# bioinformatics-centre/BayesTyper

Hardware: AMD Instinct MI355X
Metric: variant-cluster Gibbs iterations/sec + k-mer matches/sec at 1/2/4/8 MI355X (higher is better)
Workload: dtype f64 log-probabilities over u8 k-mer counts (Gibbs); u64/u8 integer (k-mer matching)

## Files before the change

bayestyper_amd/csrc/bt_gibbs.hip:

```cpp
#ifndef BT_SWEEP_OUTLINE
#define BT_SWEEP_INLINE
#endif
#include "bt_genotypes.hpp"
#include "bt_gibbs_kernel.hpp"
#include "bt_gibbs_timeline.hpp"
#include "bt_internal.hpp"

#include <algorithm>
#include <atomic>
#include <chrono>
#include <cmath>
#include <cstring>
#include <map>
#include <memory>
#include <numeric>

using namespace bt;

namespace bt {
hipError_t launch_gibbs_simple_kernel(unsigned grid, uint32_t lds, hipStream_t st, const TileDesc *tiles, uint8_t *pool, const GParams *P, int op, uint32_t a0, uint32_t a1,
                                      unsigned long long *hist, TraceCfg tr, const uint32_t *tile_list, TimelineDev *tl);
hipError_t prepare_gibbs_simple_kernel(int max_lds);
hipError_t launch_gibbs_hot_kernel(unsigned grid, unsigned block, uint32_t lds, hipStream_t st, const TileDesc *tiles, uint8_t *pool, const GParams *P, int op, uint32_t a0, uint32_t a1,
                                   unsigned long long *hist, TraceCfg tr, const uint32_t *tile_list, TimelineDev *tl);
// ... 818 lines not shown
            BT_HIP(launch_gibbs_hot_kernel(c.pack_wgs, LANES * c.pack_waves, c.pack_lds, st, g->d_tiles, g->d_pool, g->d_params, op, a0, a1, hist, tr, (const uint32_t *)c.d_pack, tl));
        else if (tl)
            hipLaunchKernelGGL(gibbs_kernel_tl, dim3((unsigned)c.tiles.size()), dim3(LANES * c.split), c.lds, st, g->d_tiles, g->d_pool, g->d_params, op, a0, a1, hist, tr,
                               (const uint32_t *)c.d_tiles, tl);
        else
            hipLaunchKernelGGL(gibbs_kernel, dim3((unsigned)c.tiles.size()), dim3(LANES * c.split), c.lds, st, g->d_tiles, g->d_pool, g->d_params, op, a0, a1, hist, tr,
                               (const uint32_t *)c.d_tiles);
        BT_CHECK_LAUNCH();
        if (tl) tl += class_waves(c);
        if (wide && c.num_fill) {
            hipLaunchKernelGGL(nan_fill_kernel, dim3(c.num_fill), dim3(256), 0, st, g->d_pool, (const FillChunk *)c.d_fill);
            BT_CHECK_LAUNCH();
        }
        if (c.stream) BT_HIP(hipEventRecord(c.done, st));
    }
    for (auto &c : g->classes)
        if (c.stream) BT_HIP(hipStreamWaitEvent(g->ctx->stream, c.done, 0));
    g->prefill_armed = wide;
    return BT_OK;
}

inline uint64_t align_up(uint64_t x, uint64_t a) { return (x + a - 1) / a * a; }
inline uint32_t tile_lds_bytes(const TileDesc &d) { return d.lds_all ? d.hot_bytes * d.nvm : d.hot_bytes; }
constexpr uint32_t kMinTileWidth = 4;
constexpr uint32_t kLightLds = 24576;
const uint32_t kClassLds[] = {16384, 32768, 0xFFFFFFFFu};

const uint32_t kElemSize[A_COUNT] = {
     1,  1,  1,  1,  4,  4,  2,  4,  2,  4,  4,  4,  2,
     1,  4,  4,  4,  2,  4,  4,  4,  4,  4,  4,
     4,  1,
     4,  8,  8,  4,  4,  4,  4,  1,  2,  8,  4,  1,
     4,  4,  4,  4,  4,  4,  8,  4,  8,  2,  8,
     8,  4,  8,  1,  4,  4,  8,  1,  1,  8,  4,  8,  4,  1,  4,  8,  4,
     4,  1,  8,  4,  4,  4,  1,  1,  1,  1,  4,  2,  4,  8,  8,  4,  2,  1,  4,  4,  4,  1,  1,  1,  1,  4,  4};

}

extern "C" {

struct bt_gibbs_source {
    bt_ctx *ctx = nullptr;
    uint32_t S = 0, G = 0, C = 0;
    std::vector<ClusterDims> cd;
    std::vector<GroupDims> gd;
    BuildBatch dev{};
// ... 326 lines not shown
            for (uint32_t c = 0; c < x.nv; ++c) cd_sel.push_back(src->cd[c0 + c]);
            gd_sel[i] = x;
        }
        C = (uint32_t)cd_sel.size();
        cd = cd_sel.data();
        gd = gd_sel.data();
    }
    if (G == 0 || C == 0) return fail("bt_gibbs_create: empty batch");
    BT_HIP(hipSetDevice(ctx->device));
    bt_gibbs *g = new bt_gibbs();
    g->ctx = ctx;
    g->G = G;
    g->C = C;
    g->S = S;
    GParams &P = g->P;
    P.S = S;
    P.seed = params->seed;
    P.num_chains = params->num_chains;
    P.burn_in = params->burn_in;
    P.num_iterations = params->num_iterations;
    P.max_hvk = params->max_haplotype_variant_kmers;
    P.noise_seeding = params->noise_seeding;
    P.rate = (double)params->kmer_subsampling_rate;
    for (uint32_t s = 0; s < S; ++s) P.gender[s] = params->gender[s] ? 1 : 0;

#define BT_TRY(x)                \
    do {                         \
        int _rc = (x);           \
        if (_rc != BT_OK) {      \
            bt_gibbs_destroy(g); \
            return _rc;          \
        }                        \
    } while (0)
#define BT_TRYHIP(x)                                                     \
    do {                                                                 \
        hipError_t _e = (x);                                             \
        if (_e != hipSuccess) {                                          \
            bt_gibbs_destroy(g);                                         \
            return fail(std::string(#x) + ": " + hipGetErrorString(_e)); \
        }                                                                \
    } while (0)

    g->h_A.assign(C, 0);
    g->h_var_off.assign((size_t)C + 1, 0);
    for (uint32_t c = 0; c < C; ++c) g->h_var_off[c + 1] = g->h_var_off[c] + cd[c].V;
    uint64_t flat_sel = 0;
// ... 2061 lines not shown
            break;
        case 2:
            for (uint64_t i = 0; i < n; ++i) h_out[i] = rng_gamma(st, nd, a[i], b[i]);
            break;
        case 3:
            for (uint64_t i = 0; i < n; ++i) h_out[i] = (double)rng_uniform_int(st, (uint32_t)a[i] + 1u);
            break;
        case 4:
            for (uint64_t i = 0; i < n; ++i) h_out[i] = rng_bernoulli(st, (double)(float)a[0]) ? 1.0 : 0.0;
            break;
        case 5: {
            std::vector<uint32_t> v((size_t)a[0]);
            for (size_t i = 0; i < v.size(); ++i) v[i] = (uint32_t)i;
            rng_shuffle_u32(st, sptr1(v.data()), (uint32_t)v.size());
            for (size_t i = 0; i < v.size(); ++i) h_out[i] = v[i];
            break;
        }
        default:
            return fail("bt_diag_rng: unknown kind");
    }
    return BT_OK;
}

}
```

bayestyper_amd/csrc/bt_gibbs_kernel.hpp:

```cpp
#pragma once
#include "bt_gibbs_tile.hpp"
#include "bt_noise_chain.hpp"
#include "bt_noise_help.hpp"
#include "bt_gibbs_simple.hpp"

namespace bt {

enum GibbsOp { OP_RUN = 0, OP_INIT_CHAIN = 1, OP_SWEEP = 2, OP_NOISE = 3, OP_RESET = 4, OP_SETUP = 5, OP_NOISE_CHAIN = 6 };

struct TraceCfg {
    uint32_t max_sweeps;
    uint32_t *counter;
    uint32_t *buf;
};

__device__ BT_NOINLINE void group_init_chain(Env env, uint32_t chain, uint32_t nvert, uint32_t nsrc, uint32_t gindex) {
    const Tile t = make_tile(env);
    const GParams BT_CAS &P = env_params(env);
    const uint32_t gseed = P.noise_seeding ? P.seed + (gindex + 1u) * (chain + 1u) : P.seed + (gindex + 1u);
    for (uint32_t v = 0; v < nvert; ++v) {
        const Vx c = make_vx(t, v);
        Env ev = env;
        const bool swap = env.resident == 0xFFFFFFFFu && t.d->hot_bytes != 0;
        if (swap) {
            hot_swap(env, v, true);
            ev.resident = v;
        }
        PROF_DECL;
        if (!make_vx(make_tile(ev), v).sc()[SC_CONSTRUCTED]) genotyper_construct(ev, v, gseed + c.cid());
        genotyper_reset(ev, v);
        if (swap) hot_swap(env, v, false);
    }
    if (nvert == 1 && nsrc == 1) return;
    uint32_t *bst = (uint32_t *)(t.base + t.d->off[A_BRNG]) + (size_t)t.plane * MT_PAD;
    mt_seed(bst, P.seed + (gindex + 1u) * (chain + 1u));
    Mt brng = mt_open(bst);
    rng_shuffle_u32(brng, t.arr<uint32_t>(A_SOURCES), nsrc);
    for (uint32_t v = 0; v < nvert; ++v) {
        const Vx c = make_vx(t, v);
        rng_shuffle_u32(brng, c.edges(), vx_ne(c));
    }
}

__device__ BT_NOINLINE void prepare_nested(Env env, uint32_t v_parent, uint32_t v_child) {
    if (env.resident != RESIDENT_ALL && env.resident != RESIDENT_NEVER) env.resident = 0xFFFFFFFFu;
    const Tile t = make_tile(env);
    const GParams BT_CAS &P = env_params(env);
    const Vx c = make_vx(t, v_parent), cc = make_vx(t, v_child);
    const uint32_t nd_n = vx_nd(c), cc_cid = cc.cid();
    const TileDesc BT_CAS &d = c.d();
    TPtr<uint32_t> ndcl = c.a<uint32_t>(A_NDCL, d.NDm > 1 ? d.NDm : 1), ndvo = c.a<uint32_t>(A_NDVOFF, d.NDm + 1);
    TPtr<uint16_t> ndv = c.a<uint16_t>(A_NDVAR, d.NDVm > 1 ? d.NDVm : 1);
    TPtr<uint32_t> pver = c.nver(), cver = cc.nver();
// ... 189 lines not shown
    const NoiseChainCtl *nc = is_nc ? (const NoiseChainCtl *)hist : nullptr;
    const bool no_lds = is_nc && (t.d->lds_all ? t.d->hot_bytes * t.d->nvm : t.d->hot_bytes) > nc->lds_cap;
    if (no_lds) env.resident = t.resident = RESIDENT_NEVER;
    const bool whole = !no_lds && (t.d->nvm == 1 || t.d->lds_all) && t.d->hot_bytes != 0 && (op == OP_RUN || op == OP_SWEEP || op == OP_INIT_CHAIN || is_nc);
    if (whole) {
        env.resident = RESIDENT_ALL;
        for (uint32_t v = 0; v < nvert; ++v) hot_swap(env, v, true);
        t.resident = RESIDENT_ALL;
        t.hot = lds_block() + t.lds0;
    }
    const bool simple = SIMPLE_ONLY;
    if (op == OP_RUN || op == OP_SWEEP || is_nc) {
        const bool is_run = op == OP_RUN;
        const uint32_t nchains = is_run ? P.num_chains : 1u;
        uint32_t n_burn = is_run ? P.burn_in : (arg1 != 0 ? 0u : arg0), n_collect = is_run ? P.num_iterations : (arg1 != 0 ? arg0 : 0u);
        if (is_nc) {
            n_burn = nc->first_collect < nc->n_iterations ? nc->first_collect : nc->n_iterations;
            n_collect = nc->n_iterations - n_burn;
            if (!nc_begin(nc)) n_burn = n_collect = 0;
        }
        for (uint32_t chain = 0; chain < nchains; ++chain) {
            if (is_run) {
                PROF_DECL;
                group_init_chain(env, chain, nvert, nsrc, gindex);
                PROF(15);
            }
            if constexpr (SIMPLE_ONLY) {
                simple_sweeps(env, t, P, n_burn, n_collect, tr.counter, tr.buf, tr.max_sweeps, tile, nc);
                if (is_run || n_collect) drain_collected(env);
            } else {
                const uint32_t i0 = is_nc ? nc->it_begin : 0u;
                for (uint32_t i = i0; i < n_burn + n_collect; ++i) {
                    if (is_nc && i > i0) {
                        nc_phase(nc, 0x10000000u | i);
                        if (!nc_wait_table(nc, i)) break;
                        if (nc->help_units) {
                            noise_help(env, nc);
                            if (!noise_help_wait(nc, tile, i)) break;
                        }
                    }
                    if (is_nc) nc_phase(nc, 0x40000000u | i);
                    const TraceRow r = trace_row_for(t, P, tr, tile);
                    if constexpr (kSingle) {
                        if (r.on)
                            for (uint32_t q = 0; q < P.S; ++q) r.row[q] = 0xFFFFFFFFu;
                        const Vx root = make_vx(t, 0);
                        TPtr<uint8_t> gploidy = t.arr<uint8_t>(A_PLOIDY);
                        for (uint32_t q = 0; q < P.S; ++q) {
                            root.nest_ploidy()[q] = gploidy[q];
                            root.nest_n()[q] = 0;
                        }
                        visit_vertex(env, t, P, 0u, i >= n_burn, r.row, r.on);
                    } else
                        group_sweep(env, t, P, i >= n_burn, nvert, nsrc, r.row, r.on);
                    if (is_nc) {
                        nc_phase(nc, 0x50000000u | i);
                        noise_tally_group(env, nvert, nc);
                        nc_phase(nc, 0x60000000u | i);
                        if (!nc_iteration_end(nc, i)) break;
                    }
                }
                if (is_run && t.d->logged) drain_collected(env);
            }
        }
        if (!simple && (is_run || n_collect))
            for (uint32_t v = 0; v < nvert; ++v) flush_vertex(env, v);
    } else if (op == OP_INIT_CHAIN) {
        group_init_chain(env, arg0, nvert, nsrc, gindex);
        if (!SIMPLE_ONLY && arg1 != 0 && wide_table(*t.d))
            for (uint32_t v = 0; v < nvert; ++v) make_vx(t, v).sc()[SC_UC_DIRTY] = 0;
    } else if (SIMPLE_ONLY) {
    } else if (op == OP_NOISE) {
        for (uint32_t v = 0; v < nvert; ++v) {
            const Vx c = make_vx(t, v);
            const uint32_t nsu = c.sc()[SC_NSUB_U];
            TPtr<uint32_t> usub = c.usub();
            for (uint32_t s = 0; s < P.S; ++s) {
                const uint16_t h1 = c.dip()[2 * s], h2 = c.dip()[2 * s + 1];
                for (uint32_t i = t.part; i < nsu; i += t.copies) {
                    const uint32_t k = usub[i];
                    if (unique_mult(c, k, h1, h2, P.gender[s]) == 0) {
                        const uint32_t cnt = c.has_counts(k) ? c.count(k, s) : 0;
                        atomicAdd(&hist[s * 256u + cnt], 1ULL);
                    }
                }
            }
            if (t.part == 0) cache_clear(c, P, false, arg0 != 0);
        }
    } else if (op == OP_RESET) {
        for (uint32_t v = 0; v < nvert; ++v) make_vx(t, v).sc()[SC_CONSTRUCTED] = 0;
    } else if (op == OP_SETUP) {
// ... 36 lines not shown
```

bayestyper_amd/csrc/bt_gibbs_tile.hpp:

```cpp
#pragma once
#include "bt_rng_device.hpp"

namespace bt {

constexpr unsigned LANES = 64;
constexpr uint16_t NOHAP = 0xFFFF;
constexpr double BT_LN2 = 0.693147180559945309417232121458176568;
constexpr double BT_DBL_EPS = 2.220446049250313080847263336181640625e-16;
#ifndef BT_LINEAR_DRAW_MIN
#define BT_LINEAR_DRAW_MIN 4u
#endif
#ifndef BT_UC_INVALIDATE_MIN
#define BT_UC_INVALIDATE_MIN 64u
#endif
#ifndef BT_EVAL_BLOCK
#define BT_EVAL_BLOCK 4u
#endif
constexpr uint32_t EVB = BT_EVAL_BLOCK;
#ifdef BT_SINGLE
constexpr bool kSingle = true;
#else
constexpr bool kSingle = false;
#endif
#ifdef BT_PACKED
// ... 120 lines not shown
    uint32_t wsh;
    uint32_t teams;
    uint32_t sblk;
};
#ifndef BT_EV_CAP
#define BT_EV_CAP 32
#endif
constexpr uint32_t EV_CAP = BT_EV_CAP;
constexpr uint32_t KSC_WAYS = 4;
constexpr uint32_t KSC_NOKEY = 0xFFFEFFFEu;
constexpr uint32_t NOHOT = 0xFFFFFFFFu;
constexpr uint32_t RESIDENT_ALL = 0xFFFFFFFEu;
constexpr uint32_t RESIDENT_NEVER = 0xFFFFFFFDu;

struct GParams {
    uint32_t S, seed, num_chains, burn_in, num_iterations, max_hvk, noise_seeding;
    double rate;
    uint8_t gender[32];
    const double BT_GAS *lut_g;
    const double BT_GAS *lut_n;
    const double BT_GAS *lgamma_int;
    const double BT_GAS *gamma_a2;
    uint32_t lgamma_n, gamma_n;
};

extern __shared__ __attribute__((aligned(16))) uint8_t bt_lds_raw[];
__device__ inline uint8_t *lds_block() { return (uint8_t *)bt_lds_raw; }
__device__ inline uint32_t pack_slot() { return blockIdx.x * (blockDim.x >> 6) + (uint32_t)__builtin_amdgcn_readfirstlane((int)(threadIdx.x >> 6)); }

__host__ __device__ constexpr bool hot_core(int a) {
    return a == A_SC || a == A_DIP || a == A_NESTPL || a == A_NESTN || a == A_KSCUPD || a == A_PEND || a == A_PENDDIP || a == A_PENDVALID || a == A_EVN || a == A_FREQ || a == A_LOGF ||
           a == A_OBS || a == A_NZ || a == A_NZLIST || a == A_UNEXT || a == A_ZHDR || a == A_ZBKT || a == A_PHDR || a == A_PBKT || a == A_RING || a == A_FNDSAVED;
}

struct Tile {
    uint8_t BT_GAS *base;
    const TileDesc BT_CAS *d;
    uint32_t lane;
    uint32_t plane;
    uint32_t part, copies;
    uint32_t wsh;
    uint8_t *hot;
    uint32_t lds0;
    uint32_t resident;
    template <typename T>
    __device__ inline SPtrF<T, LANES> harr(int a, uint32_t v, uint32_t len) const {
// ... 509 lines not shown
                uint32_t h[4], cnt[4], n = 0;
#pragma unroll
                for (int q = 0; q < 4; ++q) {
                    h[q] = 0;
                    if (word) {
                        h[q] = w * 32 + (uint32_t)__builtin_ctz(word);
                        word &= word - 1;
                        n = q + 1;
                    }
                }
#pragma unroll
                for (int q = 0; q < 4; ++q) cnt[q] = hv[h[q] * Vm + var];
#pragma unroll
                for (int q = 0; q < 4; ++q)
                    if ((uint32_t)q < n && cnt[q] < maxk) {
                        hv[h[q] * Vm + var] = cnt[q] + 1;
                        is_max = false;
                    }
            }
        }
    }
    return is_max;
}
__device__ inline void sample_kmer_subset(const Vx &c, const GParams BT_CAS &P) {
    const uint32_t Vm = c.d().Vm;
    TPtr<uint32_t> hv = c.hvcount();
    for (uint32_t h = 0; h < c.H; ++h)
        for (uint32_t v = 0; v < c.V; ++v) hv[(uint32_t)h * Vm + v] = 0;
    uint32_t nsu = 0, nsm = 0;
    MtRing rng = c.rng(0);
    TPtr<uint32_t> uniq = c.uniq(), usub = c.usub(), multi = c.multi(), msub = c.msub();
    PROF_DECL;
    const uint32_t nu = c.nu();
    rng_shuffle_u32(rng, uniq, nu);
    PROF(8);
    uint32_t nu_sel = 0, nm_sel = 0;
    for (uint32_t i = 0; i < nu; ++i)
        if (rng_bernoulli(rng, P.rate)) usub[nu_sel++] = uniq[i];
    rng_shuffle_u32(rng, multi, c.nm);
    for (uint32_t i = 0; i < c.nm; ++i)
        if (rng_bernoulli(rng, P.rate)) msub[nm_sel++] = multi[i];
    for (uint32_t i = 0; i < nu_sel; ++i) {
        const uint32_t k = usub[i];
        if (!is_max_hv_kmer(c, k, P.max_hvk)) usub[nsu++] = k;
    }
    for (uint32_t i = 0; i < nm_sel; ++i) {
        const uint32_t k = msub[i];
        if (!is_max_hv_kmer(c, k, P.max_hvk)) msub[nsm++] = k;
    }
    PROF(9);
    mt_close(rng);
    {
        const uint32_t Hm = c.d().Hm;
        const Vx::RPtr<uint8_t> sm = c.subm();
        TPtr<uint8_t> scn = c.subcnt(), sic = c.subic();
        TPtr<uint32_t> so = c.skv_off(), sb = c.skv_bits();
        TPtr<uint16_t> sv = c.skv_var();
        const uint32_t HWm = c.d().HWm, HW = (c.H + 31) / 32;
        uint32_t ne = 0;
        so[0] = 0;
        for (uint32_t i = 0; i < nsu; ++i) {
            const uint32_t k = usub[i];
            ne += c.kv_off(k + 1) - c.kv_off(k);
            so[i + 1] = ne;
        }
        for (uint32_t i = c.t.part; i < nsu; i += c.t.copies) {
            const uint32_t k = usub[i];
            uint32_t ne = so[i];
            for (uint32_t e = c.kv_off(k), e1 = c.kv_off(k + 1); e < e1; ++e, ++ne) {
                sv[ne] = c.kv_var(e);
                for (uint32_t w = 0; w < HW; ++w) sb[ne * HWm + w] = c.a<uint32_t>(A_KVBITS, c.d().NNZm * HWm)[e * HWm + w];
            }
            const bool hc = c.has_counts(k) != 0;
            {
                const Vx::RPtr<uint8_t> Mrow = c.mat(A_M, c.d().Km) + k * Hm;
                uint32_t h = 0;
                for (; h + 8 <= c.H; h += 8) {
                    uint8_t t8[8];
#pragma unroll
                    for (int q = 0; q < 8; ++q) t8[q] = Mrow[h + q];
#pragma unroll
                    for (int q = 0; q < 8; ++q) sm[i * Hm + h + q] = t8[q];
                }
                for (; h < c.H; ++h) sm[i * Hm + h] = Mrow[h];
            }
            for (uint32_t ss = 0; ss < P.S; ++ss) scn[i * P.S + ss] = hc ? c.count(k, ss) : (uint8_t)0;
            sic[2 * i] = hc ? c.ic(k, 0) : (uint8_t)0;
            sic[2 * i + 1] = hc ? c.ic(k, 1) : (uint8_t)0;
        }
    }
    {
        const uint32_t Hm = c.d().Hm;
        TPtr<uint8_t> mm = c.msubm(), mcn = c.msubc(), mic = c.msubic();
        TPtr<uint32_t> msh = c.msubsh();
        for (uint32_t i = c.t.part; i < nsm; i += c.t.copies) {
            const uint32_t k = msub[i];
            for (uint32_t h = 0; h < c.H; ++h) mm[i * Hm + h] = c.M(k, h);
            for (uint32_t ss = 0; ss < P.S; ++ss) mcn[i * P.S + ss] = c.count(k, ss);
            mic[2 * i] = c.ic(k, 0);
            mic[2 * i + 1] = c.ic(k, 1);
            msh[i] = (uint32_t)c.shared_idx(k);
        }
    }
    if (c.t.copies > 1u) copies_sync();
    PROF(10);
    SPtrF<uint32_t, LANES> sc = c.sc();
    sc[SC_NSUB_U] = nsu;
    sc[SC_NSUB_M] = nsm;
    TPtr<uint8_t> smm = c.smm(), oth = c.oth();
    for (uint32_t i = 0; i < nsm * P.S; ++i) {
        smm[i] = 0;
        oth[i] = 0;
    }
    for (uint32_t s = 0; s < P.S; ++s) c.mgen()[s] += 1;
    SPtrF<uint8_t, LANES> upd = c.ksc_upd();
    for (uint32_t s = 0; s < P.S; ++s) {
        upd[s] = 1;
        for (uint32_t e = 0; e < KSC_WAYS; ++e) c.ksc_key(s)[e] = KSC_NOKEY;
        c.ksc_key(s)[KSC_WAYS] = 0;
    }
}

__device__ BT_NOINLINE void genotyper_reset(Env env, uint32_t vtx) {
    const Vx c = make_vx(make_tile(env), vtx);
    const GParams BT_CAS &P = env_params(env);
    c.sc()[SC_USE_MULTI] = 0;
    sample_kmer_subset(c, P);
    cache_clear(c, P, true);
    freq_reset(c);
}

__device__ inline uint32_t dip_index(const Vx &c, uint16_t h1, uint16_t h2) {
    if (h2 == NOHAP) return c.H * (c.H + 1) / 2 + h1;
    return (uint32_t)h1 * c.H - ((uint32_t)h1 * ((uint32_t)h1 - 1u)) / 2u + ((uint32_t)h2 - (uint32_t)h1);
}

__device__ inline double unique_log_prob(const Vx &c, const GParams BT_CAS &P, uint32_t s, uint16_t h1, uint16_t h2, uint32_t nsub_u) {
    const TileDesc BT_CAS &d = c.d();
    const uint32_t idx = dip_index(c, h1, h2);
    uint32_t slot = 0;
    const Vx::UCPtr uc = c.ucache();
    if (d.cache_mode == 0) {
        const double v = uc[(uint32_t)s * d.Dcm + idx];
        if (v == v) return v;
    } else if (d.cache_mode == 1) {
        const uint32_t key = s * d.Dcm + idx + 1u;
        slot = hashed_slot(c, key);
        if (c.uctag()[slot] == key) return uc[slot];
    }
    double acc = 0;
// ... 1138 lines not shown
```

bayestyper_amd/csrc/bt_rng_device.hpp:

```cpp
#pragma once
#include <hip/hip_runtime.h>
#include <math.h>
#include <stdint.h>

namespace bt {

#define BT_HD __host__ __device__ inline
#if defined(BT_SIMPLE_TU) || defined(BT_SWEEP_INLINE)
#define BT_SWEEPFN inline
#else
#define BT_SWEEPFN static __noinline__
#endif
#define BT_NOINLINE static __noinline__

#if defined(__HIP_DEVICE_COMPILE__)
#define BT_MATH __host__ __device__ __noinline__
#ifdef BT_INLINE_MATH
#define BT_MATHI __host__ __device__ inline
#else
#define BT_MATHI BT_MATH
#endif
#else
#define BT_MATH __host__ __device__ inline
#define BT_MATHI BT_MATH
// ... 181 lines not shown
        } else {
            nw[4u * q] = za.x, nw[4u * q + 1u] = za.y, nw[4u * q + 2u] = za.z;
            nw[4u * q + 227u] = zb.x, nw[4u * q + 228u] = zb.y, nw[4u * q + 229u] = zb.z;
        }
        if (vc == 4u) *(MtQuadU BT_GAS *)(nw + 4u * q + 454u) = zc;
        else if (vc == 2u) nw[4u * q + 454u] = zc.x, nw[4u * q + 455u] = zc.y;
    }
    __builtin_amdgcn_fence(__ATOMIC_RELEASE, "workgroup");
    __builtin_amdgcn_wave_barrier();
    __builtin_amdgcn_fence(__ATOMIC_ACQUIRE, "workgroup");
}
__device__ static __noinline__ void mt_twist_for(bool want, uint32_t BT_GAS *st, uint32_t cur) {
    unsigned long long todo = __ballot(want);
    while (todo) {
        const int src = __builtin_ctzll(todo);
        const uint64_t p = (uint64_t)(uintptr_t)st;
        const uint32_t lo = (uint32_t)__builtin_amdgcn_readlane((int)(uint32_t)p, src), hi = (uint32_t)__builtin_amdgcn_readlane((int)(uint32_t)(p >> 32), src);
        const uint32_t c = (uint32_t)__builtin_amdgcn_readlane((int)cur, src);
        uint32_t BT_GAS *base = (uint32_t BT_GAS *)(uintptr_t)(((uint64_t)hi << 32) | lo);
        mt_twist_block(base + (c ? MT_BUF : 0u), base + (c ? 0u : MT_BUF));
        todo &= ~__ballot(want && (uint64_t)(uintptr_t)st == (((uint64_t)hi << 32) | lo));
    }
}
#endif
template <class RP>
struct MtRingT {
    uint32_t BT_GAS *st;
    RP ring;
    uint32_t cap;
    uint32_t pos, head, avail;
#ifdef BT_MT_BLOCK
    uint32_t flags = 0;
#endif
#ifdef BT_DIAG_FAKE_MT
    uint32_t fake_ctr = 0;
#endif
#if defined(BT_MT_BLOCK) && defined(__HIP_DEVICE_COMPILE__) && !defined(BT_DIAG_FAKE_MT)
    __device__ inline uint32_t BT_GAS *cur_buf() const { return st + ((flags & MT_F_CUR) ? MT_BUF : 0u); }
    __device__ inline void next_block(bool at_end) {
        mt_twist_for(at_end && !(flags & MT_F_READY), st, (flags & MT_F_CUR) ? 1u : 0u);
        if (at_end) {
            flags = (flags ^ MT_F_CUR) & ~MT_F_READY;
            pos = 0;
        }
    }
    __device__ inline void twist_ahead() {
        const bool want = pos >= MT_AHEAD && !(flags & MT_F_READY);
        if (bt_wave_any(want)) {
            mt_twist_for(want, st, (flags & MT_F_CUR) ? 1u : 0u);
            if (want) flags |= MT_F_READY;
        }
    }
    __device__ inline void chunk(bool go) {
        if (bt_wave_any(go && pos == MT_N)) next_block(go && pos == MT_N);
        if (go) {
            const MtQuad z = *(const MtQuad BT_GAS *)(cur_buf() + pos);
            const uint32_t w = (head + avail) & (cap - 1u);
            ring[w] = mt_temper(z.x);
            ring[w + 1u] = mt_temper(z.y);
            ring[w + 2u] = mt_temper(z.z);
            ring[w + 3u] = mt_temper(z.w);
            pos += 4u;
            avail += 4u;
        }
    }
    template <unsigned NB>
    __device__ inline void batch(uint32_t want) {
        if (bt_wave_any(avail < want && pos == MT_N)) next_block(avail < want && pos == MT_N);
        uint32_t nc = avail < want ? (want - avail + 3u) >> 2 : 0u;
        nc = nc < NB ? nc : NB;
        const uint32_t left = (MT_N - pos) >> 2;
        nc = nc < left ? nc : left;
        MtQuad z[NB];
        const uint32_t BT_GAS *b = cur_buf() + pos;
#pragma unroll
        for (unsigned j = 0; j < NB; ++j)
            if (j < nc) z[j] = *(const MtQuad BT_GAS *)(b + 4u * j);
        bt_sched_fence();
#pragma unroll
        for (unsigned j = 0; j < NB; ++j)
            if (j < nc) {
                const uint32_t w = (head + avail) & (cap - 1u);
                ring[w] = mt_temper(z[j].x);
                ring[w + 1u] = mt_temper(z[j].y);
                ring[w + 2u] = mt_temper(z[j].z);
                ring[w + 3u] = mt_temper(z[j].w);
                avail += 4u;
                pos += 4u;
            }
    }
    __device__ inline void fill_to(uint32_t want) {
        while (bt_wave_any(avail < want)) chunk(avail < want);
    }
    template <unsigned NB>
    __device__ inline void fill_batched(uint32_t want) {
        if (bt_wave_any(avail < want)) batch<NB>(want);
        fill_to(want);
    }
    __device__ inline void topup() {
        twist_ahead();
        fill_batched<4>(cap - 3u);
    }
#else
    BT_HD void chunk(bool go) {
#ifdef BT_DIAG_FAKE_MT
        if (go) {
            const uint32_t salt = (uint32_t)(uintptr_t)st * 2654435761u + fake_ctr;
            const uint32_t w = (head + avail) & (cap - 1u);
            for (uint32_t k = 0; k < 4u; ++k) ring[w + k] = bt_fake_word(salt + pos + k);
            fake_ctr += 0x9e3779b9u;
            pos = pos + 4u == MT_N ? 0u : pos + 4u;
            avail += 4u;
        }
        return;
#endif
        if (go) {
            const uint32_t p = pos, q = p + MT_M < MT_N ? p + MT_M : p + MT_M - MT_N;
            const MtQuad a = *(const MtQuad BT_GAS *)(st + p);
            const uint32_t a4 = st[p + 4u];
            const MtQuad b = *(const MtQuadU BT_GAS *)(st + q);
            bt_sched_fence();
            MtQuad z;
// ... 163 lines not shown
    double s1 = (double)w[2];
    s1 += (double)w[3] * 4294967296.0;
    second = s1 / 18446744073709551616.0;
    if (second >= 1.0) second = top;
}

template <class G>
BT_HD uint32_t rng_uniform_int(G &st, uint32_t range) {
    uint64_t product = (uint64_t)mt_next(st) * (uint64_t)range;
    uint32_t low = (uint32_t)product;
    if (low < range) {
        uint32_t threshold = (0u - range) % range;
        while (low < threshold) {
            product = (uint64_t)mt_next(st) * (uint64_t)range;
            low = (uint32_t)product;
        }
    }
    return (uint32_t)(product >> 32);
}

template <class G>
BT_HD bool rng_bernoulli(G &st, double p) { return rng_canonical(st) < p; }

template <class G, typename Arr>
BT_HD void rng_shuffle_u32(G &st, Arr a, uint32_t n) {
    if (n == 0) return;
    const uint64_t urngrange = 0xFFFFFFFFull;
    if (urngrange / n >= n) {
        uint32_t i = 1;
        if ((n % 2u) == 0) {
            uint32_t j = rng_uniform_int(st, 2);
            uint32_t t = a[i]; a[i] = a[j]; a[j] = t;
            ++i;
        }
        while (i != n) {
            const uint32_t swap_range = i + 1;
            const uint32_t b1 = swap_range + 1;
            uint32_t x = rng_uniform_int(st, swap_range * b1);
            uint32_t p0 = x / b1, p1 = x % b1;
            uint32_t t = a[i]; a[i] = a[p0]; a[p0] = t;
            ++i;
            t = a[i]; a[i] = a[p1]; a[p1] = t;
            ++i;
        }
        return;
    }
// ... 208 lines not shown
```

bayestyper_amd/lib.py:

```python
import ctypes as C
import os

import numpy as np

_HERE = os.path.dirname(os.path.abspath(__file__))
LIB_PATH = os.environ.get("BTGPU_LIB", os.path.join(_HERE, "libbtgpu.so"))

if not os.path.exists(LIB_PATH):
    raise ImportError(
        f"{LIB_PATH} not found: build the HIP extension first (python -c 'import __graft_entry__ as g; g.build()' "
        "or bayestyper_amd/csrc/build.sh). There is no CPU fallback."
    )

_lib = C.CDLL(LIB_PATH)

u8p, u32p, u64p, i64p, f64p, f32p = (C.POINTER(t) for t in (C.c_uint8, C.c_uint32, C.c_uint64, C.c_int64, C.c_double, C.c_float))
vp = C.c_void_p


def _sig(name, argtypes, restype=C.c_int):
    f = getattr(_lib, name)
    f.argtypes = argtypes
    f.restype = restype
    return f
# ... 603 lines not shown
bt_ctx_clone = _sig("bt_ctx_clone", [vp, C.POINTER(vp)])
bt_gibbs_reset_groups = _sig("bt_gibbs_reset_groups", [vp])
bt_gibbs_result_sizes = _sig("bt_gibbs_result_sizes", [vp, u64p, u64p])
bt_gibbs_result_fetch = _sig("bt_gibbs_result_fetch", [vp] * 7)
bt_gibbs_result_words = _sig("bt_gibbs_result_words", [vp, C.POINTER(vp), u64p])
bt_gibbs_genotypes = _sig("bt_gibbs_genotypes", [vp, vp, C.POINTER(vp), u64p])
bt_gibbs_trace_enable = _sig("bt_gibbs_trace_enable", [vp, C.c_uint32])
bt_gibbs_trace_fetch = _sig("bt_gibbs_trace_fetch", [vp, vp, C.c_uint64, u64p])
bt_gibbs_posterior_summary = _sig("bt_gibbs_posterior_summary", [vp, vp])
bt_gibbs_timeline_enable = _sig("bt_gibbs_timeline_enable", [vp, C.c_uint32])
bt_gibbs_timeline_sizes = _sig("bt_gibbs_timeline_sizes", [vp, u64p, u32p, u32p, u32p])
bt_gibbs_timeline_fetch = _sig("bt_gibbs_timeline_fetch", [vp, vp, C.c_uint64, u64p])
bt_gibbs_timeline_summary = _sig("bt_gibbs_timeline_summary", [vp, C.c_uint64, C.c_uint32, C.c_uint32, vp])
bt_gibbs_device_bytes = _sig("bt_gibbs_device_bytes", [vp, u64p])
bt_gibbs_source_create = _sig("bt_gibbs_source_create", [vp, C.c_uint32, vp, C.POINTER(vp)])
bt_gibbs_source_create_from_paths = _sig("bt_gibbs_source_create_from_paths", [vp, C.c_uint32, vp, vp, C.POINTER(vp)])
bt_gibbs_source_fetch = _sig("bt_gibbs_source_fetch", [vp, vp, vp])
bt_gibbs_source_destroy = _sig("bt_gibbs_source_destroy", [vp])
bt_gibbs_source_device_bytes = _sig("bt_gibbs_source_device_bytes", [vp, u64p])
bt_gibbs_create_from_source = _sig("bt_gibbs_create_from_source", [vp, vp, vp, vp, C.c_uint32, C.POINTER(vp)])
bt_gibbs_state_bytes_from_source = _sig("bt_gibbs_state_bytes_from_source", [vp, vp, vp, C.c_uint32, u64p])
bt_diag_uset_replay = _sig("bt_diag_uset_replay", [C.c_uint32, vp, vp, C.c_uint64, vp, u32p])
bt_diag_rng = _sig("bt_diag_rng", [C.c_uint32, C.c_int, vp, vp, C.c_uint64, vp])
bt_genotype_text_sizes = _sig("bt_genotype_text_sizes", [vp, vp, C.c_uint64, u64p, u64p])
bt_genotype_text = _sig("bt_genotype_text", [vp, vp, C.c_uint64, vp, C.c_uint64, vp, C.c_uint64, u64p, u64p, u32p])
bt_gibbs_genotype_text = _sig("bt_gibbs_genotype_text", [vp, vp, C.POINTER(vp), u64p, C.POINTER(vp), u64p, u32p])
bt_diag_genotype_text = _sig("bt_diag_genotype_text", [vp, C.c_uint64, vp, C.c_uint64, vp, C.c_uint64, u64p, u64p, u32p])
bt_diag_format_g6 = _sig("bt_diag_format_g6", [vp, C.c_uint64, vp, vp])
bt_diag_genotype_cluster = _sig("bt_diag_genotype_cluster", [C.c_uint32, C.c_uint32, C.c_uint32, vp, vp, vp, C.c_uint64, vp, vp, vp, vp, vp, vp, vp, C.c_uint64, u64p])
bt_diag_kmer_set_order = _sig("bt_diag_kmer_set_order", [vp, C.c_uint32, C.c_uint64, C.c_uint, vp, vp])
bt_diag_kmer_set_order_staged = _sig("bt_diag_kmer_set_order_staged", [vp, C.c_uint32, C.c_uint64, C.c_uint, vp, vp])
bt_kmer_set_orders = _sig("bt_kmer_set_orders", [vp, vp, vp, C.c_uint32, C.c_uint, C.c_uint64, C.c_uint32, vp, vp, vp])
bt_paths_multigroup_info = _sig("bt_paths_multigroup_info", [vp, vp])


TIMELINE_RECORD = np.dtype([("start_tick", np.uint64), ("end_tick", np.uint64), ("hw_id", np.uint32), ("xcc_id", np.uint32), ("tile", np.uint32), ("wave", np.uint32),
                            ("launch", np.uint32), ("launch_class", np.uint16), ("kernel", np.uint8), ("op", np.uint8), ("groups", np.uint32), ("lds_bytes", np.uint32)])
assert TIMELINE_RECORD.itemsize == 48
TIMELINE_KERNELS = ("general", "hot", "simple", "single")
_TIMELINE_SUMMARY_FIELDS = ("records", "unfinished", "first_start", "last_end", "busy_ticks", "peak_live", "median_end", "idle_after_median_ticks", "last_record")


def timeline_summary(records, launch=None, launch_class=None):
    records = np.ascontiguousarray(records, TIMELINE_RECORD)
    out = np.zeros(len(_TIMELINE_SUMMARY_FIELDS), np.uint64)
    check(bt_gibbs_timeline_summary(_np_ptr(records) if len(records) else None, len(records), 0xFFFFFFFF if launch is None else int(launch),
# ... 618 lines not shown
```

include/btgpu.h:

```cpp
#ifndef BTGPU_H
#define BTGPU_H

#include <stddef.h>
#include <stdint.h>

#ifdef __cplusplus
extern "C" {
#endif

#define BT_OK 0
#define BT_ERR 1

typedef struct bt_ctx bt_ctx;

const char *bt_last_error(void);
int bt_version(void);
int bt_device_count(int *count);

int bt_ctx_create(int device_id, bt_ctx **out);
int bt_ctx_clone(bt_ctx *ctx, bt_ctx **out);
int bt_ctx_destroy(bt_ctx *ctx);
int bt_ctx_set_stream(bt_ctx *ctx, void *hip_stream);
int bt_ctx_use_default_stream(bt_ctx *ctx);
int bt_sync(bt_ctx *ctx);
// ... 312 lines not shown
    uint64_t last_record;
} bt_gibbs_timeline_summary_t;
int bt_gibbs_timeline_enable(bt_gibbs *g, uint32_t max_launches);
int bt_gibbs_timeline_sizes(bt_gibbs *g, uint64_t *records, uint32_t *launches, uint32_t *dropped, uint32_t *tick_khz);
int bt_gibbs_timeline_fetch(bt_gibbs *g, bt_gibbs_timeline_record *h_out, uint64_t capacity, uint64_t *n);
int bt_gibbs_timeline_summary(const bt_gibbs_timeline_record *r, uint64_t n, uint32_t launch, uint32_t launch_class, bt_gibbs_timeline_summary_t *out);

typedef struct bt_noise_rng {
    uint32_t mt[624];
    uint32_t mt_pos;
    uint32_t saved_available;
    double saved;
} bt_noise_rng;
typedef struct bt_noise_model bt_noise_model;
int bt_noise_model_create(bt_ctx *ctx, uint32_t num_samples, const float *h_prior, bt_noise_model **out);
int bt_noise_model_destroy(bt_noise_model *m);
int bt_noise_model_set_rng(bt_noise_model *m, const bt_noise_rng *h_rng);
int bt_noise_model_get_rng(bt_noise_model *m, bt_noise_rng *h_rng);
int bt_gibbs_noise_chain(bt_gibbs *g, bt_noise_model *m, uint32_t num_iterations, uint32_t first_collect,
                         int (*reduce)(void *user, uint64_t *d_hist, uint64_t n), void *user, double *h_rates);

int bt_diag_uset_replay(uint32_t universe, const uint8_t *ops, const uint32_t *values, uint64_t num_ops, uint32_t *h_order, uint32_t *n);
int bt_diag_rng(uint32_t seed, int kind, const double *a, const double *b, uint64_t n, double *h_out);
int bt_diag_genotype_cluster(uint32_t S, uint32_t H, uint32_t V, const uint16_t *hap_allele, const uint16_t *var_num_alleles, const uint8_t *var_has_dependency,
                             uint64_t num_diplotypes, const uint16_t *h1, const uint16_t *h2, const uint32_t *freq, const double *stats, const uint8_t *ploidy,
                             const bt_genotype_filters *f, uint32_t *h_words, uint64_t capacity, uint64_t *num_words);
int bt_diag_genotype_text(const uint32_t *h_words, uint64_t num_words, uint8_t *h_text, uint64_t text_capacity, uint32_t *h_index, uint64_t index_capacity, uint64_t *text_bytes,
                          uint64_t *index_words, uint32_t *num_not_covered);
int bt_diag_format_g6(const double *h_values, uint64_t n, char *h_text16, int32_t *h_len);
int bt_diag_kmer_set_order(const uint64_t *h_kmers, uint32_t n, uint64_t initial_buckets, unsigned k, uint32_t *h_rank, uint64_t *h_final_buckets);
int bt_diag_kmer_set_order_staged(const uint64_t *h_kmers, uint32_t n, uint64_t initial_buckets, unsigned k, uint32_t *h_rank, uint64_t *h_final_buckets);

typedef struct bt_deflate_stats {
    uint64_t pieces, stored_pieces;
    uint64_t literals, matches, matched_bytes;
    uint64_t bytes_in, bytes_out;
    double seconds_h2d, seconds_kernels, seconds_d2h, seconds_host;
} bt_deflate_stats;
int bt_deflate_bound(uint64_t n, uint64_t *capacity);
int bt_deflate(bt_ctx *ctx, const uint8_t *d_in, uint64_t n, int last, uint8_t *d_out, uint64_t capacity, uint64_t *h_out_bytes, bt_deflate_stats *stats);
int bt_gzip_save(bt_ctx *ctx, const char *path, const uint8_t *h_data, uint64_t n, uint32_t threads, bt_deflate_stats *stats);
int bt_diag_deflate(const uint8_t *h_in, uint64_t n, int last, uint8_t *h_out, uint64_t capacity, uint64_t *out_bytes, bt_deflate_stats *stats);

int bt_bgzf_bound(uint64_t n, uint64_t *capacity, uint64_t *blocks);
int bt_bgzf(bt_ctx *ctx, const uint8_t *d_in, uint64_t n, int eof, uint8_t *d_out, uint64_t capacity, uint64_t *h_out_bytes, uint64_t *h_block_offsets, bt_deflate_stats *stats);
int bt_bgzf_save(bt_ctx *ctx, const char *path, const uint8_t *h_data, uint64_t n, uint32_t threads, uint64_t *h_block_offsets, uint64_t offsets_capacity, bt_deflate_stats *stats);
// ... 8 lines not shown
```

Measured before the change: 1.203 billion.

## Parallelize k-mer subset Bernoulli sampling across tile copies with bulk MT consumption

Adds a bulk Bernoulli sampler that reads Mersenne Twister words straight from the twist blocks, indexed by position. This lets the copies of a tile each evaluate a strided share of the draws and compact the selections with ballot and popcount, instead of one serial loop drawing from the RNG ring. The hv-count zeroing and per-sample cache init loops are also split across copies, and the filter step runs on part 0 with syncs around it. It is on by default through an env-controlled parameter and only affects chain initialisation in the run op. The cost is extra synchronisation and added complexity in keeping RNG state bit-exact, which a new host diagnostic entry point is meant to check.

```diff
diff --git a/bayestyper_amd/csrc/bt_gibbs.hip b/bayestyper_amd/csrc/bt_gibbs.hip
--- a/bayestyper_amd/csrc/bt_gibbs.hip
+++ b/bayestyper_amd/csrc/bt_gibbs.hip
@@ -864,6 +864,7 @@
 
 inline uint64_t align_up(uint64_t x, uint64_t a) { return (x + a - 1) / a * a; }
 inline uint32_t tile_lds_bytes(const TileDesc &d) { return d.lds_all ? d.hot_bytes * d.nvm : d.hot_bytes; }
+constexpr uint32_t kBulkSubsetDefault = 1;
 constexpr uint32_t kMinTileWidth = 4;
 constexpr uint32_t kLightLds = 24576;
 const uint32_t kClassLds[] = {16384, 32768, 0xFFFFFFFFu};
@@ -1236,6 +1237,10 @@
     P.max_hvk = params->max_haplotype_variant_kmers;
     P.noise_seeding = params->noise_seeding;
     P.rate = (double)params->kmer_subsampling_rate;
+    {
+        const char *e = getenv("BT_GIBBS_BULK_SUBSET");
+        P.bulk_subset = e ? (atoi(e) != 0 ? 1u : 0u) : kBulkSubsetDefault;
+    }
     for (uint32_t s = 0; s < S; ++s) P.gender[s] = params->gender[s] ? 1 : 0;
 
 #define BT_TRY(x)                \
@@ -3343,4 +3348,14 @@
     return BT_OK;
 }
 
-}
+int bt_diag_bulk_bernoulli(uint32_t seed, uint64_t discard, uint32_t n, double p, uint32_t ring_cap, int ahead, uint8_t *h_flags, uint32_t *h_tail, uint32_t *h_state) {
+#ifdef BT_RNG_BULK
+    if ((n && !h_flags) || !h_tail || !h_state) return fail("bt_diag_bulk_bernoulli: null argument");
+    if (ring_cap < 8 || ring_cap > 64 || (ring_cap & (ring_cap - 1u))) return fail("bt_diag_bulk_bernoulli: ring_cap must be a power of two in 8 .. 64");
+    return bulk_bernoulli_check(seed, discard, n, p, ring_cap, ahead, h_flags, h_tail, h_state), BT_OK;
+#else
+    return fail("bt_diag_bulk_bernoulli: this build has no block-form generator");
+#endif
+}
+
+}
diff --git a/bayestyper_amd/csrc/bt_gibbs_kernel.hpp b/bayestyper_amd/csrc/bt_gibbs_kernel.hpp
--- a/bayestyper_amd/csrc/bt_gibbs_kernel.hpp
+++ b/bayestyper_amd/csrc/bt_gibbs_kernel.hpp
@@ -14,7 +14,7 @@
     uint32_t *buf;
 };
 
-__device__ BT_NOINLINE void group_init_chain(Env env, uint32_t chain, uint32_t nvert, uint32_t nsrc, uint32_t gindex) {
+__device__ BT_NOINLINE void group_init_chain(Env env, uint32_t chain, uint32_t nvert, uint32_t nsrc, uint32_t gindex, bool bulk) {
     const Tile t = make_tile(env);
     const GParams BT_CAS &P = env_params(env);
     const uint32_t gseed = P.noise_seeding ? P.seed + (gindex + 1u) * (chain + 1u) : P.seed + (gindex + 1u);
@@ -28,7 +28,7 @@
         }
         PROF_DECL;
         if (!make_vx(make_tile(ev), v).sc()[SC_CONSTRUCTED]) genotyper_construct(ev, v, gseed + c.cid());
-        genotyper_reset(ev, v);
+        genotyper_reset(ev, v, bulk);
         if (swap) hot_swap(env, v, false);
     }
     if (nvert == 1 && nsrc == 1) return;
@@ -264,7 +264,7 @@
         for (uint32_t chain = 0; chain < nchains; ++chain) {
             if (is_run) {
                 PROF_DECL;
-                group_init_chain(env, chain, nvert, nsrc, gindex);
+                group_init_chain(env, chain, nvert, nsrc, gindex, P.bulk_subset != 0);
                 PROF(15);
             }
             if constexpr (SIMPLE_ONLY) {
@@ -308,7 +308,7 @@
         if (!simple && (is_run || n_collect))
             for (uint32_t v = 0; v < nvert; ++v) flush_vertex(env, v);
     } else if (op == OP_INIT_CHAIN) {
-        group_init_chain(env, arg0, nvert, nsrc, gindex);
+        group_init_chain(env, arg0, nvert, nsrc, gindex, false);
         if (!SIMPLE_ONLY && arg1 != 0 && wide_table(*t.d))
             for (uint32_t v = 0; v < nvert; ++v) make_vx(t, v).sc()[SC_UC_DIRTY] = 0;
     } else if (SIMPLE_ONLY) {
diff --git a/bayestyper_amd/csrc/bt_gibbs_tile.hpp b/bayestyper_amd/csrc/bt_gibbs_tile.hpp
--- a/bayestyper_amd/csrc/bt_gibbs_tile.hpp
+++ b/bayestyper_amd/csrc/bt_gibbs_tile.hpp
@@ -166,6 +166,7 @@
     const double BT_GAS *lgamma_int;
     const double BT_GAS *gamma_a2;
     uint32_t lgamma_n, gamma_n;
+    uint32_t bulk_subset;
 };
 
 extern __shared__ __attribute__((aligned(16))) uint8_t bt_lds_raw[];
@@ -721,11 +722,21 @@
     }
     return is_max;
 }
-__device__ inline void sample_kmer_subset(const Vx &c, const GParams BT_CAS &P) {
+__device__ inline void sample_kmer_subset(const Vx &c, const GParams BT_CAS &P, bool bulk) {
     const uint32_t Vm = c.d().Vm;
     TPtr<uint32_t> hv = c.hvcount();
-    for (uint32_t h = 0; h < c.H; ++h)
-        for (uint32_t v = 0; v < c.V; ++v) hv[(uint32_t)h * Vm + v] = 0;
+#ifdef BT_RNG_BULK
+    bulk = bulk && c.t.copies > 1u;
+#else
+    bulk = false;
+#endif
+    if (bulk) {
+        for (uint32_t h = c.t.part; h < c.H; h += c.t.copies)
+            for (uint32_t v = 0; v < c.V; ++v) hv[(uint32_t)h * Vm + v] = 0;
+    } else {
+        for (uint32_t h = 0; h < c.H; ++h)
+            for (uint32_t v = 0; v < c.V; ++v) hv[(uint32_t)h * Vm + v] = 0;
+    }
     uint32_t nsu = 0, nsm = 0;
     MtRing rng = c.rng(0);
     TPtr<uint32_t> uniq = c.uniq(), usub = c.usub(), multi = c.multi(), msub = c.msub();
@@ -734,18 +745,58 @@
     rng_shuffle_u32(rng, uniq, nu);
     PROF(8);
     uint32_t nu_sel = 0, nm_sel = 0;
-    for (uint32_t i = 0; i < nu; ++i)
-        if (rng_bernoulli(rng, P.rate)) usub[nu_sel++] = uniq[i];
-    rng_shuffle_u32(rng, multi, c.nm);
-    for (uint32_t i = 0; i < c.nm; ++i)
-        if (rng_bernoulli(rng, P.rate)) msub[nm_sel++] = multi[i];
-    for (uint32_t i = 0; i < nu_sel; ++i) {
-        const uint32_t k = usub[i];
-        if (!is_max_hv_kmer(c, k, P.max_hvk)) usub[nsu++] = k;
-    }
-    for (uint32_t i = 0; i < nm_sel; ++i) {
-        const uint32_t k = msub[i];
-        if (!is_max_hv_kmer(c, k, P.max_hvk)) msub[nsm++] = k;
+#ifdef BT_RNG_BULK
+    if (bulk) {
+        const MtTeamCopies team(c.t.part, c.t.copies);
+        rng_bernoulli_bulk(rng, nu, P.rate, team, [&](uint32_t i, bool sel, unsigned long long b) {
+            if (sel) usub[nu_sel + team.below(b)] = uniq[i];
+            nu_sel += (uint32_t)__popcll(b);
+        });
+        rng_shuffle_u32(rng, multi, c.nm);
+        rng_bernoulli_bulk(rng, c.nm, P.rate, team, [&](uint32_t i, bool sel, unsigned long long b) {
+            if (sel) msub[nm_sel + team.below(b)] = multi[i];
+            nm_sel += (uint32_t)__popcll(b);
+        });
+        copies_sync();
+        SPtrF<uint32_t, LANES> sc = c.sc();
+        if (c.t.part == 0) {
+            TPtr<uint32_t> so = c.skv_off();
+            uint32_t ne = 0;
+            so[0] = 0;
+            for (uint32_t i = 0; i < nu_sel; ++i) {
+                const uint32_t k = usub[i];
+                if (!is_max_hv_kmer(c, k, P.max_hvk)) {
+                    usub[nsu++] = k;
+                    ne += c.kv_off(k + 1) - c.kv_off(k);
+                    so[nsu] = ne;
+                }
+            }
+            for (uint32_t i = 0; i < nm_sel; ++i) {
+                const uint32_t k = msub[i];
+                if (!is_max_hv_kmer(c, k, P.max_hvk)) msub[nsm++] = k;
+            }
+            sc[SC_NSUB_U] = nsu;
+            sc[SC_NSUB_M] = nsm;
+        }
+        copies_sync();
+        nsu = sc[SC_NSUB_U];
+        nsm = sc[SC_NSUB_M];
+    } else
+#endif
+    {
+        for (uint32_t i = 0; i < nu; ++i)
+            if (rng_bernoulli(rng, P.rate)) usub[nu_sel++] = uniq[i];
+        rng_shuffle_u32(rng, multi, c.nm);
+        for (uint32_t i = 0; i < c.nm; ++i)
+            if (rng_bernoulli(rng, P.rate)) msub[nm_sel++] = multi[i];
+        for (uint32_t i = 0; i < nu_sel; ++i) {
+            const uint32_t k = usub[i];
+            if (!is_max_hv_kmer(c, k, P.max_hvk)) usub[nsu++] = k;
+        }
+        for (uint32_t i = 0; i < nm_sel; ++i) {
+            const uint32_t k = msub[i];
+            if (!is_max_hv_kmer(c, k, P.max_hvk)) msub[nsm++] = k;
+        }
     }
     PROF(9);
     mt_close(rng);
@@ -756,12 +807,14 @@
         TPtr<uint32_t> so = c.skv_off(), sb = c.skv_bits();
         TPtr<uint16_t> sv = c.skv_var();
         const uint32_t HWm = c.d().HWm, HW = (c.H + 31) / 32;
-        uint32_t ne = 0;
-        so[0] = 0;
-        for (uint32_t i = 0; i < nsu; ++i) {
-            const uint32_t k = usub[i];
-            ne += c.kv_off(k + 1) - c.kv_off(k);
-            so[i + 1] = ne;
+        if (!bulk) {
+            uint32_t ne = 0;
+            so[0] = 0;
+            for (uint32_t i = 0; i < nsu; ++i) {
+                const uint32_t k = usub[i];
+                ne += c.kv_off(k + 1) - c.kv_off(k);
+                so[i + 1] = ne;
+            }
         }
         for (uint32_t i = c.t.part; i < nsu; i += c.t.copies) {
             const uint32_t k = usub[i];
@@ -807,24 +860,25 @@
     sc[SC_NSUB_U] = nsu;
     sc[SC_NSUB_M] = nsm;
     TPtr<uint8_t> smm = c.smm(), oth = c.oth();
-    for (uint32_t i = 0; i < nsm * P.S; ++i) {
+    for (uint32_t i = bulk ? c.t.part : 0u, step = bulk ? c.t.copies : 1u; i < nsm * P.S; i += step) {
         smm[i] = 0;
         oth[i] = 0;
     }
     for (uint32_t s = 0; s < P.S; ++s) c.mgen()[s] += 1;
     SPtrF<uint8_t, LANES> upd = c.ksc_upd();
-    for (uint32_t s = 0; s < P.S; ++s) {
+    for (uint32_t s = bulk ? c.t.part : 0u, step = bulk ? c.t.copies : 1u; s < P.S; s += step) {
         upd[s] = 1;
         for (uint32_t e = 0; e < KSC_WAYS; ++e) c.ksc_key(s)[e] = KSC_NOKEY;
         c.ksc_key(s)[KSC_WAYS] = 0;
     }
-}
-
-__device__ BT_NOINLINE void genotyper_reset(Env env, uint32_t vtx) {
+    if (bulk) copies_sync();
+}
+
+__device__ BT_NOINLINE void genotyper_reset(Env env, uint32_t vtx, bool bulk) {
     const Vx c = make_vx(make_tile(env), vtx);
     const GParams BT_CAS &P = env_params(env);
     c.sc()[SC_USE_MULTI] = 0;
-    sample_kmer_subset(c, P);
+    sample_kmer_subset(c, P, bulk);
     cache_clear(c, P, true);
     freq_reset(c);
 }
diff --git a/bayestyper_amd/csrc/bt_rng_device.hpp b/bayestyper_amd/csrc/bt_rng_device.hpp
--- a/bayestyper_amd/csrc/bt_rng_device.hpp
+++ b/bayestyper_amd/csrc/bt_rng_device.hpp
@@ -227,6 +227,13 @@
         todo &= ~__ballot(want && (uint64_t)(uintptr_t)st == (((uint64_t)hi << 32) | lo));
     }
 }
+#else
+inline void mt_twist_block(const uint32_t *old, uint32_t *nw) {
+    for (uint32_t i = 0; i < MT_N; ++i) nw[i] = mt_twist(old[i], i + 1u < MT_N ? old[i + 1u] : nw[0], i < MT_N - MT_M ? old[i + MT_M] : nw[i - (MT_N - MT_M)]);
+}
+inline void mt_twist_for(bool want, uint32_t *st, uint32_t cur) {
+    if (want) mt_twist_block(st + (cur ? MT_BUF : 0u), st + (cur ? 0u : MT_BUF));
+}
 #endif
 template <class RP>
 struct MtRingT {
@@ -240,23 +247,23 @@
 #ifdef BT_DIAG_FAKE_MT
     uint32_t fake_ctr = 0;
 #endif
-#if defined(BT_MT_BLOCK) && defined(__HIP_DEVICE_COMPILE__) && !defined(BT_DIAG_FAKE_MT)
-    __device__ inline uint32_t BT_GAS *cur_buf() const { return st + ((flags & MT_F_CUR) ? MT_BUF : 0u); }
-    __device__ inline void next_block(bool at_end) {
+#if defined(BT_MT_BLOCK) && !defined(BT_DIAG_FAKE_MT)
+    BT_HD uint32_t BT_GAS *cur_buf() const { return st + ((flags & MT_F_CUR) ? MT_BUF : 0u); }
+    BT_HD void next_block(bool at_end) {
         mt_twist_for(at_end && !(flags & MT_F_READY), st, (flags & MT_F_CUR) ? 1u : 0u);
         if (at_end) {
             flags = (flags ^ MT_F_CUR) & ~MT_F_READY;
             pos = 0;
         }
     }
-    __device__ inline void twist_ahead() {
+    BT_HD void twist_ahead() {
         const bool want = pos >= MT_AHEAD && !(flags & MT_F_READY);
         if (bt_wave_any(want)) {
             mt_twist_for(want, st, (flags & MT_F_CUR) ? 1u : 0u);
             if (want) flags |= MT_F_READY;
         }
     }
-    __device__ inline void chunk(bool go) {
+    BT_HD void chunk(bool go) {
         if (bt_wave_any(go && pos == MT_N)) next_block(go && pos == MT_N);
         if (go) {
             const MtQuad z = *(const MtQuad BT_GAS *)(cur_buf() + pos);
@@ -270,7 +277,7 @@
         }
     }
     template <unsigned NB>
-    __device__ inline void batch(uint32_t want) {
+    BT_HD void batch(uint32_t want) {
         if (bt_wave_any(avail < want && pos == MT_N)) next_block(avail < want && pos == MT_N);
         uint32_t nc = avail < want ? (want - avail + 3u) >> 2 : 0u;
         nc = nc < NB ? nc : NB;
@@ -294,15 +301,15 @@
                 pos += 4u;
             }
     }
-    __device__ inline void fill_to(uint32_t want) {
+    BT_HD void fill_to(uint32_t want) {
         while (bt_wave_any(avail < want)) chunk(avail < want);
     }
     template <unsigned NB>
-    __device__ inline void fill_batched(uint32_t want) {
+    BT_HD void fill_batched(uint32_t want) {
         if (bt_wave_any(avail < want)) batch<NB>(want);
         fill_to(want);
     }
-    __device__ inline void topup() {
+    BT_HD void topup() {
         twist_ahead();
         fill_batched<4>(cap - 3u);
     }
@@ -512,6 +519,122 @@
 template <class G>
 BT_HD bool rng_bernoulli(G &st, double p) { return rng_canonical(st) < p; }
 
+#if defined(BT_MT_BLOCK) && !defined(BT_DIAG_FAKE_MT)
+#define BT_RNG_BULK 1
+struct MtTeamOne {
+    BT_HD uint32_t rank() const { return 0u; }
+    BT_HD uint32_t size() const { return 1u; }
+    BT_HD unsigned long long ballot(bool f) const { return f ? 1ull : 0ull; }
+    BT_HD uint32_t below(unsigned long long) const { return 0u; }
+    BT_HD bool any(bool f) const { return f; }
+    BT_HD void sync() const {}
+};
+struct MtTeamCopies {
+    uint32_t part, copies;
+    unsigned long long gmask, lower;
+    __device__ inline MtTeamCopies(uint32_t part_, uint32_t copies_) : part(part_), copies(copies_) {
+        const uint32_t lane = threadIdx.x & 63u, width = 64u / copies_;
+        unsigned long long m = 0;
+        for (uint32_t k = 0; k < copies_; ++k) m |= 1ull << (lane % width + k * width);
+        gmask = m;
+        lower = (1ull << lane) - 1ull;
+    }
+    __device__ inline uint32_t rank() const { return part; }
+    __device__ inline uint32_t size() const { return copies; }
+    __device__ inline unsigned long long ballot(bool f) const { return __ballot(f) & gmask; }
+    __device__ inline uint32_t below(unsigned long long b) const { return (uint32_t)__popcll(b & lower); }
+    __device__ inline bool any(bool f) const { return bt_wave_any(f); }
+    __device__ inline void sync() const {
+        __builtin_amdgcn_fence(__ATOMIC_RELEASE, "workgroup");
+        __builtin_amdgcn_wave_barrier();
+        __builtin_amdgcn_fence(__ATOMIC_ACQUIRE, "workgroup");
+    }
+};
+template <class G, class T, class F>
+BT_HD void rng_bernoulli_bulk(G &m, uint32_t n, double p, const T &team, F &&emit) {
+    const uint32_t a0 = m.avail, h0 = m.head, p0 = m.pos, mask = m.cap - 1u, cur0 = (m.flags & MT_F_CUR) ? 1u : 0u;
+    const bool ready0 = (m.flags & MT_F_READY) != 0;
+    uint32_t produced = 0;
+    if (n > (a0 >> 1)) {
+        const uint32_t want = m.cap - 3u < 16u ? m.cap - 3u : 16u;
+        const uint32_t add = ((want - (a0 & 1u) + 3u) >> 2) << 2, per = add >> 1;
+        produced = (n - (a0 >> 1) + per - 1u) / per * add;
+    }
+    const uint32_t blocks = produced ? (p0 + produced - 1u) / MT_N : 0u;
+    auto word = [&](uint32_t j) -> uint32_t {
+        if (j < a0) return m.ring[(h0 + j) & mask];
+        const uint32_t q = p0 + (j - a0), k = q / MT_N;
+        return mt_temper(m.st[(((cur0 + k) & 1u) ? MT_BUF : 0u) + (q - k * MT_N)]);
+    };
+    uint32_t lo = 0;
+    for (uint32_t k = 0; team.any(k <= blocks); ++k) {
+        const bool live = k <= blocks;
+        if (k) mt_twist_for(live && !(k == 1u && ready0), m.st, (cur0 + k - 1u) & 1u);
+        uint32_t hi = (a0 + MT_N * (k + 1u) - p0) >> 1;
+        hi = hi < n ? hi : n;
+        for (uint32_t base = lo; team.any(live && base < hi); base += team.size()) {
+            const uint32_t i = base + team.rank();
+            const bool in = live && i < hi;
+            bool sel = false;
+            if (in) {
+                double sum = (double)word(2u * i);
+                sum += (double)word(2u * i + 1u) * 4294967296.0;
+                double u = sum / 18446744073709551616.0;
+                if (u >= 1.0) u = 0.99999999999999988897769753748434595763683319091796875;
+                sel = u < p;
+            }
+            const unsigned long long b = team.ballot(sel);
+            if (live && base < hi) emit(i, sel, b);
+        }
+        if (live) lo = hi;
+    }
+    const uint32_t end = a0 + produced;
+    for (uint32_t j = (2u * n > a0 ? 2u * n : a0) + team.rank(); j < end; j += team.size()) m.ring[(h0 + j) & mask] = word(j);
+    team.sync();
+    m.head = (h0 + 2u * n) & mask;
+    m.avail = end - 2u * n;
+    m.pos = p0 + produced - blocks * MT_N;
+    if (blocks) m.flags = (cur0 ^ (blocks & 1u)) ? MT_F_CUR : 0u;
+}
+__host__ inline void bulk_bernoulli_check(uint32_t seed, uint64_t discard, uint32_t n, double p, uint32_t ring_cap, int ahead, uint8_t *flags, uint32_t *tail, uint32_t *state) {
+    typedef SPtrF<uint32_t, 1> RP;
+    uint32_t *st0 = new uint32_t[2 * MT_BUF](), *ring0 = new uint32_t[ring_cap + MT_RING_HDR]();
+    uint32_t *st = new uint32_t[2 * MT_BUF], *ring = new uint32_t[ring_cap + MT_RING_HDR], *dst = new uint32_t[MT_WORDS];
+    mt_ring_seed(st0, RP{ring0, 0u, 0u}, ring_cap, seed);
+    {
+        MtRing m = mt_ring_open(st0, RP{ring0, 0u, 0u}, ring_cap);
+        for (uint64_t i = 0; i < discard; ++i) (void)m.next();
+        if (ahead) m.twist_ahead();
+        mt_close(m);
+    }
+    for (uint32_t form = 0; form < 2; ++form) {
+        for (uint32_t i = 0; i < 2 * MT_BUF; ++i) st[i] = st0[i];
+        for (uint32_t i = 0; i < ring_cap + MT_RING_HDR; ++i) ring[i] = ring0[i];
+        MtRing m = mt_ring_open(st, RP{ring, 0u, 0u}, ring_cap);
+        uint8_t *f = flags + (size_t)form * n;
+        if (form == 0) {
+            for (uint32_t i = 0; i < n; ++i) f[i] = rng_bernoulli(m, p) ? 1 : 0;
+        } else {
+            for (uint32_t i = 0; i < n; ++i) f[i] = 0xFF;
+            const MtTeamOne team;
+            rng_bernoulli_bulk(m, n, p, team, [&](uint32_t i, bool sel, unsigned long long) { f[i] = sel ? 1 : 0; });
+        }
+        state[4 * form] = m.pos, state[4 * form + 1] = m.flags, state[4 * form + 2] = m.head, state[4 * form + 3] = m.avail;
+        for (uint32_t k = 0; k < 8; ++k) tail[8 * form + k] = m.next();
+    }
+    mt_seed(dst, seed);
+    Mt d = mt_open(dst);
+    for (uint64_t i = 0; i < discard; ++i) (void)d.next();
+    for (uint32_t i = 0; i < n; ++i) flags[2 * (size_t)n + i] = rng_bernoulli(d, p) ? 1 : 0;
+    for (uint32_t k = 0; k < 8; ++k) tail[16 + k] = d.next();
+    delete[] st0;
+    delete[] ring0;
+    delete[] st;
+    delete[] ring;
+    delete[] dst;
+}
+#endif
+
 template <class G, typename Arr>
 BT_HD void rng_shuffle_u32(G &st, Arr a, uint32_t n) {
     if (n == 0) return;
diff --git a/bayestyper_amd/lib.py b/bayestyper_amd/lib.py
--- a/bayestyper_amd/lib.py
+++ b/bayestyper_amd/lib.py
@@ -649,6 +649,7 @@
 bt_gibbs_state_bytes_from_source = _sig("bt_gibbs_state_bytes_from_source", [vp, vp, vp, C.c_uint32, u64p])
 bt_diag_uset_replay = _sig("bt_diag_uset_replay", [C.c_uint32, vp, vp, C.c_uint64, vp, u32p])
 bt_diag_rng = _sig("bt_diag_rng", [C.c_uint32, C.c_int, vp, vp, C.c_uint64, vp])
+bt_diag_bulk_bernoulli = _sig("bt_diag_bulk_bernoulli", [C.c_uint32, C.c_uint64, C.c_uint32, C.c_double, C.c_uint32, C.c_int, vp, vp, vp])
 bt_genotype_text_sizes = _sig("bt_genotype_text_sizes", [vp, vp, C.c_uint64, u64p, u64p])
 bt_genotype_text = _sig("bt_genotype_text", [vp, vp, C.c_uint64, vp, C.c_uint64, vp, C.c_uint64, u64p, u64p, u32p])
 bt_gibbs_genotype_text = _sig("bt_gibbs_genotype_text", [vp, vp, C.POINTER(vp), u64p, C.POINTER(vp), u64p, u32p])
diff --git a/include/btgpu.h b/include/btgpu.h
--- a/include/btgpu.h
+++ b/include/btgpu.h
@@ -358,6 +358,7 @@
 
 int bt_diag_uset_replay(uint32_t universe, const uint8_t *ops, const uint32_t *values, uint64_t num_ops, uint32_t *h_order, uint32_t *n);
 int bt_diag_rng(uint32_t seed, int kind, const double *a, const double *b, uint64_t n, double *h_out);
+int bt_diag_bulk_bernoulli(uint32_t seed, uint64_t discard, uint32_t n, double p, uint32_t ring_cap, int ahead, uint8_t *h_flags, uint32_t *h_tail, uint32_t *h_state);
 int bt_diag_genotype_cluster(uint32_t S, uint32_t H, uint32_t V, const uint16_t *hap_allele, const uint16_t *var_num_alleles, const uint8_t *var_has_dependency,
                              uint64_t num_diplotypes, const uint16_t *h1, const uint16_t *h2, const uint32_t *freq, const double *stats, const uint8_t *ploidy,
                              const bt_genotype_filters *f, uint32_t *h_words, uint64_t capacity, uint64_t *num_words);
```

Measured after the change: 1.243 billion, median of 6. 1.03x the previous value.
